# flash4242/Promptable-Counterfactual-GAN

Hardware: AMD Instinct MI355X
Metric: images/sec (G+D step) MNIST-28 cDCGAN bs512 @1/2/4/8 MI355X; % MFMA roofline (higher is better)
Workload: dtype f32

## Files before the change

### promptable-counterfactual-gan_amd/csrc/conv_igemm.hip

```cpp
#include <string.h>
#include <array>
#include <map>
#include <mutex>
#include "conv_loaders.h"
#include "conv_pixtab.h"
#include "conv_cliptab.h"
#include "thin_conv.h"

namespace pcg {
namespace {

__device__ __forceinline__ int wave_id() { return __builtin_amdgcn_readfirstlane((int)(threadIdx.x >> 6)); }

__device__ __forceinline__ void prio_entry(const ConvP& p) { if (p.edge_prio & 1) __builtin_amdgcn_s_setprio(3); }
__device__ __forceinline__ void prio_epilogue(const ConvP& p) { if (p.edge_prio & 2) __builtin_amdgcn_s_setprio(3); }

__device__ __forceinline__ int epi_group_off(const ConvP& p, int m_block) {
  return p.epi.group_rows > 0 ? __builtin_amdgcn_readfirstlane(m_block / p.epi.group_rows) * p.N : 0;
}

template <class Cfg, bool XF, bool CLIP = false>
__global__ void __launch_bounds__(IG_THREADS, Cfg::MINW) conv_fwd_kernel(ConvP p) {
  extern __shared__ __attribute__((aligned(16))) float smem[];
  prio_entry(p);
// ... 1782 lines not shown
      const int M = g->B * g->OH * g->OW, N = g->KH * g->KW * g->Cin, kt = ceil_div(g->Cout, IG_BK), tiles = ceil_div(M, 128) * ceil_div(N, 128);
      SkPlan sk{};
      say("%s", "GEMM + col2im: ");
      if (have && plan_sk_shape(tiles, kt, &sk)) say("stream-K: %d whole tiles + %d tiles x %d k-tiles over %d ranges", sk.dp_tiles, sk.sk_tiles, kt, sk.sk_blocks);
      else say("128x128 tiles: %d", tiles);
    } else {
      DgradPhases ph{};
      int maxMp = 0;
      const int nph = build_phases(g, &ph, &maxMp);
      const int N = g->Cin, tilesN = ceil_div(N, N > 64 ? 128 : 64);
      bool uniform = true;
      for (int i = 0; i < nph; ++i)
        uniform = uniform && ph.p[i].Mp == ph.p[0].Mp && ph.p[i].nth * ph.p[i].ntw == ph.p[0].nth * ph.p[0].ntw && ph.p[i].nth > 0 && ph.p[i].ntw > 0;
      SkNPlan sn{};
      SkPlan sk{};
      say("%d phase%s: ", nph, nph == 1 ? "" : "s");
      if (N > 64 && have && !uniform && plan_skn_shape(ph, nph, 128, tilesN, g->Cout, &sn))
        say("stream-K over unequal phases: %d tiles, %d k-tile iterations over %d ranges", sn.tile0[nph], sn.total, sn.blocks);
      else if (N > 64 && have && uniform && nph > 0 &&
               plan_sk_shape(ceil_div(maxMp, 128) * tilesN * nph, ph.p[0].nth * ph.p[0].ntw * ceil_div(g->Cout, IG_BK), &sk))
        say("stream-K: %d whole tiles + %d tiles over %d ranges", sk.dp_tiles, sk.sk_tiles, sk.sk_blocks);
      else say("%s tiles: %d per phase", N > 64 ? "128x128" : "128x64", ceil_div(maxMp, 128) * tilesN);
    }
  } else {
    const WgradPlan w = plan_wgrad(g);
    SkPlan sk{};
    if (!w.narrow && !w.wide192 && w.tiles > 96 && have && plan_sk_shape(w.tiles, w.ktiles_total, &sk))
      say("stream-K: %d whole tiles + %d tiles x %d k-tiles over %d ranges, dw written by the epilogue", sk.dp_tiles, sk.sk_tiles, w.ktiles_total, sk.sk_blocks);
    else if (!w.narrow && !w.wide192 && w.tiles > 96 && w.splits == 1 && sk_mode() != 0) say("128x128 tiles: %d, dw written by the epilogue", w.tiles);
    else say("%s tiles: %d x %d K-slices of %d k-tiles (slabs + slab_reduce)", w.wide192 ? "64x192" : w.narrow ? "64x128" : "128x128", w.tiles, w.splits, w.ktiles_per_split);
  }
  snprintf(out, out_bytes, "%s", buf);
  return PCG_OK;
}

extern "C" int pcg_conv_pad_clip_query(const pcg_conv_geom* g, int32_t op, int32_t groups, int32_t assume_scratch, int32_t* taken,
                                       int32_t* order, int32_t* tile_rows, double* predicted) {
  if (int e = check_geom(g)) return e;
  PCG_REQUIRE((op == 0 || op == 1) && groups >= 1, "pcg_conv_pad_clip_query: bad arguments");
  const int have = assume_scratch && sk_mode() != 0 ? 1 : 0;
  ClipPlan cp{false, 0, 0, 1.0};
  if (mfma_layer(g) && op == 0) {
    const int M = g->B * g->OH * g->OW, N = g->Cout, kt = g->KH * g->KW * ceil_div(g->Cin, IG_BK);
    const FwdPlan f = plan_fwd(g, have);
    const bool t64 = fwd_use_t64(M, N, f.splits);
    SkPlan sk{};
    const bool plain = f.splits == 1 && !(N > 64 && !t64 && have && plan_sk_shape(ceil_div(M, 128) * ceil_div(N, 128), kt, &sk));
    cp = clip_fwd_plan(g, groups, t64, plain);
  } else if (mfma_layer(g) && g->stride <= 2 && !dgrad_as_gemm(g, have)) {
    DgradPhases ph{};
    int maxMp = 0;
    const int nph = build_phases(g, &ph, &maxMp);
    SkPlan sk{};
    const bool plain = nph == 4 && !(g->Cin > 64 && have && plan_sk_shape(ceil_div(maxMp, 128) * ceil_div(g->Cin, 128) * nph, 4 * ceil_div(g->Cout, IG_BK), &sk));
    const uint32_t w_bytes = (uint32_t)((int64_t)g->Cout * g->KH * g->KW * g->Cin * 4);
    cp = clip_dgrad_plan(g, groups, dgrad_interleaved(w_bytes, ph, nph), plain);
  }
  if (taken) *taken = cp.take && cliptab_of(g) ? 1 : 0;
  if (order) *order = cp.order;
  if (tile_rows) *tile_rows = cp.bm;
  if (predicted) *predicted = cp.ratio;
  return PCG_OK;
}

extern "C" int pcg_tune_set(const char* name, int32_t value) {
  PCG_REQUIRE(name != nullptr, "pcg_tune_set: null name");
  if (!strcmp(name, "korder")) g_tune.korder = value;
  else if (!strcmp(name, "edge_prio")) g_tune.edge_prio = value;
  else if (!strcmp(name, "dgrad_swz3")) g_tune.dgrad_swz3 = value;
  else if (!strcmp(name, "wgrad_rounds")) g_tune.wgrad_rounds = value;
  else if (!strcmp(name, "wgrad_order")) g_tune.wgrad_order = value;
  else if (!strcmp(name, "dgrad_interleave")) g_tune.dgrad_interleave = value;
  else if (!strcmp(name, "fwd_splits")) g_tune.fwd_splits = value;
  else if (!strcmp(name, "stream_k")) g_tune.stream_k = value;
  else if (!strcmp(name, "sk_blocks")) g_tune.sk_blocks = value;
  else if (!strcmp(name, "dgrad_gemm")) g_tune.dgrad_gemm = value;
  else if (!strcmp(name, "t64")) g_tune.t64 = value;
  else if (!strcmp(name, "wgrad_pixtab")) g_tune.wgrad_pixtab = value;
  else if (!strcmp(name, "pad_clip")) g_tune.pad_clip = value;
  else if (!strcmp(name, "pad_clip_dgrad")) {
    PCG_REQUIRE(value >= -1 && value <= 2, "pcg_tune_set: pad_clip_dgrad is 0, 1 or 2 (-1: built-in), not %d", (int)value);
    g_tune.pad_clip_dgrad = value;
  }
  else {
    set_error("pcg_tune_set: unknown switch '%s' (korder, edge_prio, dgrad_swz3, wgrad_rounds, wgrad_order, dgrad_interleave, fwd_splits, "
              "stream_k, sk_blocks, dgrad_gemm, t64); the loader switches wgrad_pixtab, pad_clip and pad_clip_dgrad are accepted as well", name);
    return PCG_ERR_INVALID;
  }
  return PCG_OK;
}

extern "C" int pcg_debug_stamp_buffer(void* buf, int64_t bytes) {
  g_tune.stamps = static_cast<unsigned long long*>(buf);
  g_tune.stamp_slots = buf ? (int)(bytes / 16) : 0;
#ifdef PCG_CLOCK_STAMP
  return 1;
#else
  return 0;
#endif
}
```

### promptable-counterfactual-gan_amd/csrc/thin_conv.h

```cpp
#pragma once
#include "pcg_common.h"

namespace pcg {

inline bool thin_is_cin(const pcg_conv_geom* g) { return g->Cin <= 3; }
inline bool thin_is_cout(const pcg_conv_geom* g) { return g->Cout <= 3 && !thin_is_cin(g); }

struct ThinBnIn { const float* mean; const float* invstd; const float* gamma; const float* beta; int act; float slope; int groups; };
bool thin_conv_bnin_full_ok(const pcg_conv_geom* g, int groups);
int thin_conv_fwd(const pcg_conv_geom* g, const float* x, const float* w, const float* bias, float* y, void* ws,
                  size_t ws_bytes, hipStream_t s, int act = PCG_ACT_NONE, float slope = 0.f, const ThinBnIn* bnin = nullptr);
struct ThinXf { const float* scale; const float* shift; float neg; };
bool thin_conv_xf_ok(const pcg_conv_geom* g);
int thin_conv_dgrad(const pcg_conv_geom* g, const float* dy, const float* w, const float* bias_x, float* dx, void* ws,
                    size_t ws_bytes, hipStream_t s, int act = PCG_ACT_NONE, float slope = 0.f, const ThinXf* xf = nullptr);
size_t thin_conv_fwd_workspace_bytes(const pcg_conv_geom* g);
size_t thin_conv_dgrad_workspace_bytes(const pcg_conv_geom* g);
size_t thin_conv_wgrad_workspace_bytes(const pcg_conv_geom* g);
int thin_conv_wgrad(const pcg_conv_geom* g, const float* x, const float* dy, float* dw, int accumulate, void* ws,
                    size_t ws_bytes, hipStream_t s, const ThinXf* xf = nullptr, const ThinBnIn* bnin = nullptr);

bool thin_conv_fwd_bnbwd_ok(const pcg_conv_geom* g);
size_t thin_conv_fwd_bnbwd_workspace_bytes(const pcg_conv_geom* g);
int thin_conv_fwd_bnbwd(const pcg_conv_geom* g, const float* x, const float* w, const float* z, const float* mean, const float* invstd,
                        const float* gamma, const float* beta, int act, float slope, float* dz, float* dgamma, float* dbeta, int accumulate,
                        void* ws, size_t ws_bytes, hipStream_t s);

bool thin_conv_dgrad_mask_ok(const pcg_conv_geom* g);
int thin_conv_dgrad_mask(const pcg_conv_geom* g, const float* dy, const float* w, const float* a_below, int act, float slope, float* dx,
                         hipStream_t s);

bool thin_conv_dgrad_bnbwd_full_ok(const pcg_conv_geom* g, int groups);
size_t thin_conv_dgrad_bnbwd_full_workspace_bytes(const pcg_conv_geom* g, int groups);
int thin_conv_dgrad_bnbwd_full(const pcg_conv_geom* g, const float* dy, const float* w, const float* z, const float* mean, const float* invstd,
                               const float* gamma, const float* beta, int act, float slope, float* dz, float* dgamma, float* dbeta, int accumulate,
                               int groups, void* ws, size_t ws_bytes, hipStream_t s);

int launch_slab_reduce(const float* slab, float* dw, size_t n, size_t slab_stride, int nslabs, int accumulate, hipStream_t s, bool deferrable = false);

int slab_defer_begin(hipStream_t s);
int slab_defer_flush(hipStream_t s);
int slab_defer_pending();

}
```

### promptable-counterfactual-gan_amd/csrc/thin_conv.hip

```cpp
#include "thin_conv.h"
#include <cstdlib>

namespace pcg {
namespace {

struct ThinP {
  const float* thin;
  const float* wide;
  const float* w;
  const float* bias;
  float* out;
  int act; float slope;
  const float* xf_scale; const float* xf_shift; float xf_neg;
  const float* mask_src; float mask_neg;
  int B, TH, TW, Cs, WH, WW, C;
  int KH, KW, stride, pad, transposed;
  int wsS, wsT, wsC;
  int IH_, IW_;
  int QH, QW;
  int npix;
  FastDiv dIW, dIH, dCQ;
};

__device__ __forceinline__ bool tap_map(const ThinP& p, int ph, int pw, int kh, int kw, int& qh, int& qw) {
  if (!p.transposed) {
    qh = ph * p.stride - p.pad + kh;
    qw = pw * p.stride - p.pad + kw;
  } else {
    const int th = ph + p.pad - kh, tw = pw + p.pad - kw;
    if (th < 0 || tw < 0) return false;
    if (p.stride == 1) { qh = th; qw = tw; }
    else if (p.stride == 2) { if ((th | tw) & 1) return false; qh = th >> 1; qw = tw >> 1; }
    else { if (th % p.stride || tw % p.stride) return false; qh = th / p.stride; qw = tw / p.stride; }
  }
  return (unsigned)qh < (unsigned)p.QH && (unsigned)qw < (unsigned)p.QW;
}

__device__ __forceinline__ void stage_weights(const ThinP& p, float* Wl) {
  const int TT = p.KH * p.KW * p.Cs;
  for (int i = threadIdx.x; i < TT * p.C; i += blockDim.x) {
    const int t = i / p.C, c = i - t * p.C;
    const int tap = t / p.Cs, cs = t - tap * p.Cs;
    Wl[i] = p.w[(size_t)cs * p.wsS + (size_t)tap * p.wsT + (size_t)c * p.wsC];
  }
  __syncthreads();
}

__global__ void __launch_bounds__(256) thin_expand_kernel(ThinP p) {
  extern __shared__ __attribute__((aligned(16))) float Wl[];
  stage_weights(p, Wl);
  const int CQ = p.C >> 2;
  const uint32_t total = (uint32_t)p.npix * (uint32_t)CQ;
  const float4* bias4 = reinterpret_cast<const float4*>(p.bias);
  float4* out4 = reinterpret_cast<float4*>(p.out);
  for (uint32_t idx = blockIdx.x * 256u + threadIdx.x; idx < total; idx += gridDim.x * 256u) {
    uint32_t pix, cq, t, pw, b, ph;
    p.dCQ.divmod(idx, pix, cq);
    p.dIW.divmod(pix, t, pw);
    p.dIH.divmod(t, b, ph);
    float4 acc = p.bias ? bias4[cq] : make_float4(0.f, 0.f, 0.f, 0.f);
    for (int kh = 0; kh < p.KH; ++kh)
      for (int kw = 0; kw < p.KW; ++kw) {
        int qh, qw;
        if (!tap_map(p, (int)ph, (int)pw, kh, kw, qh, qw)) continue;
        const float* sp = p.thin + (size_t)(((int)b * p.TH + qh) * p.TW + qw) * p.Cs;
        const float* wl = Wl + (size_t)((kh * p.KW + kw) * p.Cs) * p.C + 4 * cq;
        for (int cs = 0; cs < p.Cs; ++cs) {
          const float sv = sp[cs];
          const float4 w4 = *reinterpret_cast<const float4*>(wl + (size_t)cs * p.C);
          acc.x = fmaf(sv, w4.x, acc.x); acc.y = fmaf(sv, w4.y, acc.y);
          acc.z = fmaf(sv, w4.z, acc.z); acc.w = fmaf(sv, w4.w, acc.w);
        }
      }
    if (p.act != PCG_ACT_NONE) {
      acc.x = act_neg_scale(acc.x, p.slope); acc.y = act_neg_scale(acc.y, p.slope);
      acc.z = act_neg_scale(acc.z, p.slope); acc.w = act_neg_scale(acc.w, p.slope);
    }
    out4[idx] = acc;
  }
}

__global__ void __launch_bounds__(256) thin_reduce_kernel(ThinP p) {
  extern __shared__ __attribute__((aligned(16))) float Wl[];
  stage_weights(p, Wl);
  const int CQ = p.C >> 2;
  const int l16 = threadIdx.x & 15, grp = threadIdx.x >> 4;
  for (uint32_t pix = blockIdx.x * 16u + grp; pix < (uint32_t)p.npix; pix += gridDim.x * 16u) {
// ... 429 lines not shown
}

bool is_pow2(int v) { return v > 0 && (v & (v - 1)) == 0; }

bool rows_plan(const ThinP& p, RowsP& rp, size_t* patch_bytes, int px_per_thread = 16, size_t max_patch_bytes = (size_t)ROWS_MAXP * 256 * sizeof(float)) {
  const bool direct = !p.transposed;
  if (!direct && p.stride != 1) return false;
  const int CQ = p.C / 4;
  if (p.C % 4 || CQ > 256 || !is_pow2(CQ)) return false;
  if (p.IH_ * p.IW_ < 64) return false;
  if ((int64_t)p.B * p.TH * p.TW * p.Cs * 4 >= (1ll << 31)) return false;
  const int PL = 256 / CQ;
  int R;
  if (px_per_thread == 16) {
    int target = PL * 16;
    if (target < 256) target = 256;
    R = (target + p.IW_ - 1) / p.IW_;
  } else {
    R = PL * px_per_thread / p.IW_;
    if (R < 1) return false;
  }
  if (R > p.IH_) R = p.IH_;
  rp.s = direct ? p.stride : 1;
  rp.flip = direct ? 0 : 1;
  rp.qh_off = direct ? -p.pad : p.pad - p.KH + 1;
  rp.qw_off = direct ? -p.pad : p.pad - p.KW + 1;
  rp.R = R;
  rp.upi = (p.IH_ + R - 1) / R;
  rp.nunits = p.B * rp.upi;
  rp.PH = (R - 1) * rp.s + p.KH;
  rp.PW = (p.IW_ - 1) * rp.s + p.KW;
  rp.dUPI = FastDiv((uint32_t)rp.upi);
  rp.dPWC = FastDiv((uint32_t)(rp.PW * p.Cs));
  rp.dCS = FastDiv((uint32_t)p.Cs);
  *patch_bytes = (size_t)rp.PH * rp.PW * p.Cs * sizeof(float);
  return *patch_bytes <= max_patch_bytes;
}

int fill_common(ThinP& p, const pcg_conv_geom* g, bool cin_thin, bool iter_on_output) {
  p.B = g->B; p.KH = g->KH; p.KW = g->KW; p.stride = g->stride; p.pad = g->pad;
  const int T = g->KH * g->KW;
  if (cin_thin) {
    p.TH = g->IH; p.TW = g->IW; p.Cs = g->Cin; p.WH = g->OH; p.WW = g->OW; p.C = g->Cout;
    p.wsS = 1; p.wsT = g->Cin; p.wsC = T * g->Cin;
  } else {
    p.TH = g->OH; p.TW = g->OW; p.Cs = g->Cout; p.WH = g->IH; p.WW = g->IW; p.C = g->Cin;
    p.wsS = T * g->Cin; p.wsT = g->Cin; p.wsC = 1;
  }
  p.transposed = iter_on_output ? 0 : 1;
  if (iter_on_output) { p.IH_ = g->OH; p.IW_ = g->OW; p.QH = g->IH; p.QW = g->IW; }
  else { p.IH_ = g->IH; p.IW_ = g->IW; p.QH = g->OH; p.QW = g->OW; }
  p.npix = g->B * p.IH_ * p.IW_;
  p.dIW = FastDiv((uint32_t)p.IW_); p.dIH = FastDiv((uint32_t)p.IH_); p.dCQ = FastDiv((uint32_t)(p.C / 4));
  PCG_REQUIRE(p.C % 4 == 0, "thin conv: wide channel count %d must be a multiple of 4", p.C);
  PCG_REQUIRE(p.Cs >= 1 && p.Cs <= 3, "thin conv: thin channel count %d not in 1..3", p.Cs);
  PCG_REQUIRE((int64_t)p.npix * (p.C / 4) < (1ll << 31), "thin conv: problem too large for 32-bit indexing");
  return PCG_OK;
}

unsigned rows_expand_blocks(int nunits) {
  static const int cap = [] { const char* e = getenv("PCG_ROWS_EXPAND_BLOCKS"); const int v = e ? atoi(e) : 0; return v > 0 ? v : 1024; }();
  return (unsigned)(nunits < cap ? nunits : cap);
}

size_t lds_weight_bytes(const ThinP& p) { return (size_t)p.KH * p.KW * p.Cs * p.C * sizeof(float); }

bool fast_ok(const ThinP& p) {
  return p.Cs == 1 && p.stride <= 2 && p.KH * p.KW <= 16 && p.C % 16 == 0 && lds_weight_bytes(p) <= 64 * 1024;
}

int launch_expand(ThinP& p, hipStream_t s) {
  const size_t smem = lds_weight_bytes(p);
  PCG_REQUIRE(smem <= 64 * 1024, "thin conv: weight image %zu B exceeds 64 KB of LDS", smem);
  const bool k44 = p.KH == 4 && p.KW == 4, k33 = p.KH == 3 && p.KW == 3, k11 = p.KH == 1 && p.KW == 1;
  RowsP rp{};
  size_t patch_bytes = 0;
  if ((k44 || k33) && (k33 || p.Cs == 1) && rows_plan(p, rp, &patch_bytes)) {
    const size_t two = 2 * ((patch_bytes + 15) & ~(size_t)15), sm = smem > two ? smem : two;
    const uint32_t thin_bytes = (uint32_t)((int64_t)p.B * p.TH * p.TW * p.Cs * 4);
    const unsigned blocks = rows_expand_blocks(rp.nunits);
    static const int mfma_on = [] { const char* e = getenv("PCG_EXPAND_MFMA"); return e ? atoi(e) : 1; }();
    if (mfma_on && p.C == 64 && (((uintptr_t)p.out | (uintptr_t)p.mask_src) & 15) == 0) {
      const size_t sm2 = 2 * ((patch_bytes + 15) & ~(size_t)15);
      if (k44) hipLaunchKernelGGL((thin_rows_expand_mfma_kernel<4, 4, 1>), dim3(blocks), dim3(256), sm2, s, p, rp, thin_bytes);
      else if (p.Cs == 1) hipLaunchKernelGGL((thin_rows_expand_mfma_kernel<3, 3, 1>), dim3(blocks), dim3(256), sm2, s, p, rp, thin_bytes);
      else if (p.Cs == 2) hipLaunchKernelGGL((thin_rows_expand_mfma_kernel<3, 3, 2>), dim3(blocks), dim3(256), sm2, s, p, rp, thin_bytes);
      else hipLaunchKernelGGL((thin_rows_expand_mfma_kernel<3, 3, 3>), dim3(blocks), dim3(256), sm2, s, p, rp, thin_bytes);
      return launch_status("thin_rows_expand_mfma_kernel");
    }
#define PCG_ROWS_EXPAND_CASE(KH_, KW_, CS_)                                                                                  \
    if (p.KH == KH_ && p.Cs == CS_) {                                                                                         \
      hipLaunchKernelGGL((thin_rows_expand_kernel<KH_, KW_, CS_>), dim3(blocks), dim3(256), sm, s, p, rp, thin_bytes);      \
      return launch_status("thin_rows_expand_kernel");                                                                        \
    }
    PCG_ROWS_EXPAND_CASE(4, 4, 1)
    PCG_ROWS_EXPAND_CASE(3, 3, 1)
    PCG_ROWS_EXPAND_CASE(3, 3, 2)
    PCG_ROWS_EXPAND_CASE(3, 3, 3)
#undef PCG_ROWS_EXPAND_CASE
  }
  if (fast_ok(p) && (k44 || k33 || k11) && (int64_t)p.npix * (p.C / 16) < (1ll << 31)) {
    ThinP q = p;
    q.dCQ = FastDiv((uint32_t)(p.C / 16));
    const uint32_t thin_bytes = (uint32_t)((int64_t)p.B * p.TH * p.TW * 4);
    const uint64_t total = (uint64_t)p.npix * (p.C / 16);
    unsigned blocks = (unsigned)((total + 255) / 256);
    if (blocks > 8192) blocks = 8192;
    if (k44) hipLaunchKernelGGL((thin_expand16_kernel<4, 4>), dim3(blocks), dim3(256), smem, s, q, thin_bytes);
    else if (k33) hipLaunchKernelGGL((thin_expand16_kernel<3, 3>), dim3(blocks), dim3(256), smem, s, q, thin_bytes);
    else hipLaunchKernelGGL((thin_expand16_kernel<1, 1>), dim3(blocks), dim3(256), smem, s, q, thin_bytes);
    return launch_status("thin_expand16_kernel");
  }
  const uint64_t total = (uint64_t)p.npix * (p.C / 4);
  unsigned blocks = (unsigned)((total + 255) / 256);
  if (blocks > 4096) blocks = 4096;
  hipLaunchKernelGGL(thin_expand_kernel, dim3(blocks), dim3(256), smem, s, p);
  return launch_status("thin_expand_kernel");
}

bool fast32_ok(const ThinP& p) {
  return p.Cs >= 2 && p.Cs <= 3 && p.KH == 3 && p.KW == 3 && p.stride <= 2 && p.C % 16 == 0 && lds_weight_bytes(p) <= 64 * 1024;
}

size_t reduce_scratch_bytes(const ThinP& p) {
  if (fast32_ok(p)) {
    const int64_t b = (int64_t)p.B * p.WH * p.WW * 32 * 4;
    return b < (1ll << 31) ? (size_t)b : 0;
  }
  if (!fast_ok(p)) return 0;
  const int64_t b = (int64_t)p.B * p.WH * p.WW * 16 * 4;
  return b < (1ll << 31) ? (size_t)b : 0;
}

int launch_reduce(ThinP& p, void* ws, size_t ws_bytes, hipStream_t s) {
  const size_t smem = lds_weight_bytes(p);
  PCG_REQUIRE(smem <= 64 * 1024, "thin conv: weight image %zu B exceeds 64 KB of LDS", smem);
  const size_t need = reduce_scratch_bytes(p);
  PCG_REQUIRE(!p.xf_scale || !fast32_ok(p), "thin conv: input transforms only with one thin channel");
  if (need && ws && ws_bytes >= need && (((uintptr_t)ws) & 15) == 0 && fast32_ok(p)) {
    float* T = (float*)ws;
    ThinP q = p;
    q.npix = p.B * p.WH * p.WW;
    unsigned blocks = (unsigned)((q.npix + 15) / 16);
    if (blocks > 8192) blocks = 8192;
    uint32_t plane = 0;
    if (p.C == 64 && (((uintptr_t)p.wide) & 15) == 0) {
      unsigned mb = (unsigned)((q.npix + 127) / 128);
      if (mb > 4096) mb = 4096;
      hipLaunchKernelGGL((thin_tapdot64_mfma_kernel<2, false>), dim3(mb), dim3(256), 0, s, q, T);
      plane = (uint32_t)q.npix;
    } else if (p.Cs == 2) hipLaunchKernelGGL(thin_tapdot32_kernel<18>, dim3(blocks), dim3(256), smem, s, q, T);
    else hipLaunchKernelGGL(thin_tapdot32_kernel<27>, dim3(blocks), dim3(256), smem, s, q, T);
    if (int e = launch_status("thin_tapdot32_kernel")) return e;
    unsigned b2 = (unsigned)(((int64_t)p.npix * p.Cs + 255) / 256);
    if (b2 > 8192) b2 = 8192;
    hipLaunchKernelGGL(thin_col2im32_kernel, dim3(b2), dim3(256), 0, s, p, (const float*)T, (uint32_t)need, plane);
    return launch_status("thin_col2im32_kernel");
  }
  if (need && ws && ws_bytes >= need && (((uintptr_t)ws) & 15) == 0) {
    float* T = (float*)ws;
    ThinP q = p;
    q.npix = p.B * p.WH * p.WW;
    unsigned blocks = (unsigned)((q.npix + 15) / 16);
    if (blocks > 8192) blocks = 8192;
    const int nt = p.KH * p.KW;
    const bool mfma1 = p.C == 64, mfmaN = p.C % 64 == 0 && p.C > 64 && p.C <= TD64_MAX_C;
    uint32_t plane = 0;
    PCG_REQUIRE(!p.xf_scale || ((mfma1 || mfmaN) && nt <= 16 && (((uintptr_t)p.wide) & 15) == 0), "thin conv: an input transform needs the matrix-core tap-dot form");
    if ((mfma1 || mfmaN) && nt <= 16 && (((uintptr_t)p.wide) & 15) == 0) {
      unsigned mb = (unsigned)((q.npix + 127) / 128);
      if (mb > 4096) mb = 4096;
      if (mfma1) hipLaunchKernelGGL((thin_tapdot64_mfma_kernel<1, false>), dim3(mb), dim3(256), 0, s, q, T);
      else {
        if (mb > 1024) mb = 1024;
        hipLaunchKernelGGL((thin_tapdot64_mfma_kernel<1, true>), dim3(mb), dim3(256), (size_t)16 * (p.C + 4) * sizeof(float), s, q, T);
      }
      plane = (uint32_t)q.npix;
    } else if (nt == 16) hipLaunchKernelGGL(thin_tapdot_kernel<16>, dim3(blocks), dim3(256), smem, s, q, T);
    else if (nt == 9) hipLaunchKernelGGL(thin_tapdot_kernel<9>, dim3(blocks), dim3(256), smem, s, q, T);
    else if (nt == 1) hipLaunchKernelGGL(thin_tapdot_kernel<1>, dim3(blocks), dim3(256), smem, s, q, T);
    else goto generic;
    if (int e = launch_status("thin_tapdot_kernel")) return e;
    if (p.transposed && p.stride == 2 && p.KH == 4 && p.KW == 4 && p.IW_ % 4 == 0 && (((uintptr_t)p.out) & 15) == 0) {
      unsigned b4 = (unsigned)((p.npix / 4 + 255) / 256);
      if (b4 > 8192) b4 = 8192;
      hipLaunchKernelGGL(thin_col2im_s2k4_kernel, dim3(b4), dim3(256), 0, s, p, (const float*)T, (uint32_t)need, plane);
      return launch_status("thin_col2im_s2k4_kernel");
    }
    unsigned b2 = (unsigned)((p.npix + 255) / 256);
    if (b2 > 8192) b2 = 8192;
    hipLaunchKernelGGL(thin_col2im_kernel, dim3(b2), dim3(256), 0, s, p, (const float*)T, (uint32_t)need, plane);
    return launch_status("thin_col2im_kernel");
  }
generic:
  PCG_REQUIRE(!p.xf_scale, "thin conv: an input transform needs the matrix-core tap-dot form (workspace of pcg_conv2d_dgrad_workspace_bytes)");
  unsigned blocks = (unsigned)((p.npix + 15) / 16);
  if (blocks > 4096) blocks = 4096;
  hipLaunchKernelGGL(thin_reduce_kernel, dim3(blocks), dim3(256), smem, s, p);
  return launch_status("thin_reduce_kernel");
}

int rows_wgrad_blocks(const RowsP& rp) { return rp.nunits < 512 ? rp.nunits : 512; }
bool rows_wgrad_ok(const ThinP& p, const pcg_conv_geom* g, RowsP& rp, size_t* patch_bytes) {
  const bool k44 = g->KH == 4 && g->KW == 4 && p.Cs == 1, k33 = g->KH == 3 && g->KW == 3;
  return (k44 || k33) && rows_plan(p, rp, patch_bytes, ROWS_NPT, (size_t)ROWS_MAXP * 256 * sizeof(float));
}

struct ThinWgradPlan { int ppb, nblocks; };
ThinWgradPlan plan_thin_wgrad(int npix, int C) {
  ThinWgradPlan w;
  const int PL = 256 / (C / 4);
  int ppb = (npix + 1023) / 1024;
  const int min_ppb = PL * 8;
  if (ppb < min_ppb) ppb = min_ppb;
  w.ppb = ppb;
  w.nblocks = (npix + ppb - 1) / ppb;
  return w;
}

bool thin_wgrad_instantiated(const ThinP& p) {
  const bool k44 = p.KH == 4 && p.KW == 4, k33 = p.KH == 3 && p.KW == 3, k11 = p.KH == 1 && p.KW == 1;
  return p.C / 4 <= 256 && is_pow2(p.C / 4) && ((k44 && p.Cs == 1) || k33 || k11) && !(p.transposed && p.stride > 2);
}
ThinWgradPlan plan_thin_wgrad_any(int npix) {
  ThinWgradPlan w;
  int ppb = (npix + 1023) / 1024;
  if (ppb < 256) ppb = 256;
  w.ppb = ppb;
  w.nblocks = (npix + ppb - 1) / ppb;
  return w;
}

}

int launch_slab_reduce(const float* slab, float* dw, size_t n, size_t slab_stride, int nslabs, int accumulate, hipStream_t s, bool deferrable) {
  const bool vec = (n % 4 == 0) && (slab_stride % 4 == 0) && (((uintptr_t)slab | (uintptr_t)dw) & 15) == 0;
  if (deferrable && vec && g_slab_defer.on && s == g_slab_defer.stream && n / 4 < (1ull << 32) && slab_stride / 4 < (1ull << 32)) {
    SlabDefer& d = g_slab_defer;
    const size_t n4 = n / 4;
    bool clash = d.n == SLAB_MANY_MAX;
    for (int k = 0; k < d.n && !clash; ++k) clash = (const void*)d.m.e[k].dw == (const void*)dw;
    if (clash)
      if (int e = slab_defer_launch()) return e;
    const int wide = nslabs >= 64 && n4 <= 16 * 1024;
    d.m.e[d.n++] = SlabEntry{reinterpret_cast<const float4*>(slab), reinterpret_cast<float4*>(dw), (uint32_t)n4, (uint32_t)(slab_stride / 4), nslabs,
                             accumulate, wide};
    const unsigned blocks = (unsigned)(wide ? (n4 + 15) / 16 : (n4 + 255) / 256);
    if (blocks > d.max_blocks) d.max_blocks = blocks;
    return PCG_OK;
  }
  if (vec) {
    const size_t n4 = n / 4;
    if (nslabs >= 64 && n4 <= 16 * 1024) {
      hipLaunchKernelGGL(slab_reduce4_wide_kernel, dim3((unsigned)((n4 + 15) / 16)), dim3(256), 0, s, reinterpret_cast<const float4*>(slab),
                         reinterpret_cast<float4*>(dw), n4, slab_stride / 4, nslabs, accumulate);
      return launch_status("slab_reduce_kernel");
    }
    unsigned blocks = (unsigned)((n4 + 63) / 64);
    if (blocks > 4096) blocks = 4096;
    if (blocks == 0) blocks = 1;
    hipLaunchKernelGGL(slab_reduce4_kernel, dim3(blocks), dim3(64), 0, s, reinterpret_cast<const float4*>(slab),
                       reinterpret_cast<float4*>(dw), n4, slab_stride / 4, nslabs, accumulate);
  } else {
    unsigned blocks = (unsigned)((n + 255) / 256);
    if (blocks > 2048) blocks = 2048;
    if (blocks == 0) blocks = 1;
    hipLaunchKernelGGL(slab_reduce1_kernel, dim3(blocks), dim3(256), 0, s, slab, dw, n, slab_stride, nslabs, accumulate);
  }
  return launch_status("slab_reduce_kernel");
}

bool thin_conv_bnin_full_ok(const pcg_conv_geom* g, int groups) {
  if (!full_window(g) || groups < 1 || groups > 8 || g->B % groups || g->Cin % 4) return false;
  const int CQ = g->Cin / 4;
  return CQ <= 256 && 256 % CQ == 0 && (g->B / groups) % FULL_ROWS_DW == 0;
}
static FullXf full_xf_of(const pcg_conv_geom* g, const ThinBnIn* bi) {
  if (!bi || !bi->mean) return FullXf{nullptr, nullptr, nullptr, nullptr, 1.f, g->Cin, g->B};
  return FullXf{bi->mean, bi->invstd, bi->gamma, bi->beta, act_neg_of(bi->act, bi->slope), g->Cin, g->B / bi->groups};
}

int thin_conv_fwd(const pcg_conv_geom* g, const float* x, const float* w, const float* bias, float* y, void* ws,
                  size_t ws_bytes, hipStream_t s, int act, float slope, const ThinBnIn* bnin) {
  PCG_REQUIRE(!(bnin && bnin->mean) || (thin_conv_bnin_full_ok(g, bnin->groups) && (((uintptr_t)x | (uintptr_t)w) & 15) == 0),
              "thin conv forward: a BatchNorm input needs the full-window form (thin_conv_bnin_full_ok) and 16-byte aligned tensors");
  ThinP p{};
  p.act = act; p.slope = slope;
  const bool cin_thin = thin_is_cin(g);
  if (int e = fill_common(p, g, cin_thin, true)) return e;
  p.w = w; p.bias = bias; p.out = y;
  if (cin_thin) {
    p.thin = x;
    const bool fuse = act_is_cheap(act);
    p.act = fuse ? act : PCG_ACT_NONE; p.slope = act_neg_of(p.act, slope);
    if (int e = launch_expand(p, s)) return e;
    return fuse ? PCG_OK : pcg_act_fwd(y, (int64_t)g->B * g->OH * g->OW * g->Cout, act, slope, y, (pcg_stream_t)s);
  }
  p.wide = x;
  if (full_window(g) && (((uintptr_t)x | (uintptr_t)w) & 15) == 0) {
    const int L4 = g->KH * g->KW * g->Cin / 4;
    hipLaunchKernelGGL(thin_full_dot_kernel, dim3((unsigned)(g->B < 4096 ? g->B : 4096)), dim3(256), 0, s, reinterpret_cast<const float4*>(x),
                       reinterpret_cast<const float4*>(w), bias, y, g->B, L4, act, slope, full_xf_of(g, bnin));
    return launch_status("thin_full_dot_kernel");
  }
  return launch_reduce(p, ws, ws_bytes, s);
}

int launch_bn_bwd_finalize(const double* partial, int nblocks, int64_t rows, int C, const float* gamma, const float* invstd, float* coef,
                           float* dgamma, float* dbeta, int accumulate, hipStream_t s);

constexpr unsigned THIN_BN_BLOCKS = 2048;
size_t thin_conv_fwd_bnbwd_workspace_bytes(const pcg_conv_geom* g) {
  return (size_t)THIN_BN_BLOCKS * 2 * g->Cout * sizeof(double) + (size_t)3 * g->Cout * sizeof(float);
}
bool thin_conv_fwd_bnbwd_ok(const pcg_conv_geom* g) {
  if (!thin_is_cin(g) || g->Cin != 1 || !(g->KH == 4 && g->KW == 4)) return false;
  ThinP p{};
// ... 265 lines not shown
```

### promptable-counterfactual-gan_amd/csrc/thin_rows.inc

```

struct RowsP {
  int R, upi, nunits;
  int PH, PW;
  int s;
  int qh_off, qw_off;
  int flip;
  FastDiv dUPI, dPWC, dCS;
};

constexpr int ROWS_MAXP = 8;
struct PatchGather { int pr[ROWS_MAXP], pc[ROWS_MAXP]; };
__device__ __forceinline__ void patch_gather_init(const RowsP& rp, int PF, PatchGather& pg) {
#pragma unroll
  for (int j = 0; j < ROWS_MAXP; ++j) {
    const int i = threadIdx.x + 256 * j;
    uint32_t r, rem, c, cs;
    rp.dPWC.divmod((uint32_t)i, r, rem);
    rp.dCS.divmod(rem, c, cs);
    pg.pr[j] = i < PF ? (int)r : -(1 << 20);
    pg.pc[j] = ((rp.qw_off + (int)c) << 2) | (int)cs;
  }
}
template <int CS>
__device__ __forceinline__ void patch_issue(const ThinP& p, const RowsP& rp, thin_rsrc_t rs, const PatchGather& pg, int b, int r0,
// ... 17 lines not shown
template <int KH, int KW, int CS>
__global__ void __launch_bounds__(256) thin_rows_expand_kernel(ThinP p, RowsP rp, uint32_t thin_bytes) {
  constexpr int NT = KH * KW * CS;
  extern __shared__ __attribute__((aligned(16))) float smem_rows[];
  float* Wl = smem_rows;
  const int CQ = p.C >> 2, PL = 256 / CQ;
  const int cq = threadIdx.x % CQ, pl = threadIdx.x / CQ;
  for (int i = threadIdx.x; i < NT * p.C; i += 256) {
    const int t = i / p.C, c = i - t * p.C;
    const int tap = t / CS, cs = t - tap * CS;
    Wl[i] = p.w[(size_t)cs * p.wsS + (size_t)tap * p.wsT + (size_t)c * p.wsC];
  }
  __syncthreads();
  float4 w[NT];
#pragma unroll
  for (int t = 0; t < NT; ++t) w[t] = *reinterpret_cast<const float4*>(Wl + t * p.C + 4 * cq);
  const float4 bv = p.bias ? *reinterpret_cast<const float4*>(p.bias + 4 * cq) : make_float4(0.f, 0.f, 0.f, 0.f);
  const thin_rsrc_t rs = thin_rsrc(p.thin, thin_bytes);
  const FastDiv dIW = p.dIW;
  const int PF = rp.PH * rp.PW * CS, PFS = (PF + 3) & ~3;
  PatchGather pg;
  patch_gather_init(rp, PF, pg);
  float pv[ROWS_MAXP];
  int cur = 0;
  if ((int)blockIdx.x < rp.nunits) {
    uint32_t b, ur;
    rp.dUPI.divmod(blockIdx.x, b, ur);
    patch_issue<CS>(p, rp, rs, pg, (int)b, (int)ur * rp.R, pv);
  }
  __syncthreads();
  patch_put(smem_rows, pv, PF);
  __syncthreads();
  for (int unit = blockIdx.x; unit < rp.nunits; unit += gridDim.x) {
    uint32_t b, ur;
    rp.dUPI.divmod((uint32_t)unit, b, ur);
    const int r0 = (int)ur * rp.R;
    const int nxt = unit + (int)gridDim.x;
    if (nxt < rp.nunits) {
      uint32_t bn_, un_;
      rp.dUPI.divmod((uint32_t)nxt, bn_, un_);
      patch_issue<CS>(p, rp, rs, pg, (int)bn_, (int)un_ * rp.R, pv);
    }
    const float* patch = smem_rows + cur * PFS;
    int rows = p.IH_ - r0; if (rows > rp.R) rows = rp.R;
    const int np = rows * p.IW_;
    float4* o = reinterpret_cast<float4*>(p.out + ((size_t)((int)b * p.IH_ + r0) * p.IW_) * p.C) + cq;
    const float4* ms = p.mask_src ? reinterpret_cast<const float4*>(p.mask_src + ((size_t)((int)b * p.IH_ + r0) * p.IW_) * p.C) + cq : nullptr;
    for (int lp = pl; lp < np; lp += PL) {
      float4 mv = make_float4(1.f, 1.f, 1.f, 1.f);
      if (ms) mv = ms[(size_t)lp * CQ];
      uint32_t lh, pw;
      dIW.divmod((uint32_t)lp, lh, pw);
      const float* pp = patch + ((int)lh * rp.s * rp.PW + (int)pw * rp.s) * CS;
      float4 acc = bv;
#pragma unroll
      for (int kh = 0; kh < KH; ++kh)
#pragma unroll
        for (int kw = 0; kw < KW; ++kw) {
          const int khp = rp.flip ? KH - 1 - kh : kh, kwp = rp.flip ? KW - 1 - kw : kw;
#pragma unroll
          for (int cs = 0; cs < CS; ++cs) {
            const float sv = pp[(khp * rp.PW + kwp) * CS + cs];
            const float4 w4 = w[(kh * KW + kw) * CS + cs];
            acc.x = fmaf(sv, w4.x, acc.x); acc.y = fmaf(sv, w4.y, acc.y);
            acc.z = fmaf(sv, w4.z, acc.z); acc.w = fmaf(sv, w4.w, acc.w);
          }
        }
      if (p.act != PCG_ACT_NONE) {
        acc.x = act_neg_scale(acc.x, p.slope); acc.y = act_neg_scale(acc.y, p.slope);
        acc.z = act_neg_scale(acc.z, p.slope); acc.w = act_neg_scale(acc.w, p.slope);
      }
      if (ms) {
        acc.x *= mv.x > 0.f ? 1.f : p.mask_neg; acc.y *= mv.y > 0.f ? 1.f : p.mask_neg;
        acc.z *= mv.z > 0.f ? 1.f : p.mask_neg; acc.w *= mv.w > 0.f ? 1.f : p.mask_neg;
      }
      o[(size_t)lp * CQ] = acc;
    }
    if (nxt < rp.nunits) patch_put(smem_rows + (cur ^ 1) * PFS, pv, PF);
    __syncthreads();
    cur ^= 1;
  }
}

template <int KH, int KW, int CS>
__global__ void __launch_bounds__(256) thin_rows_expand_mfma_kernel(ThinP p, RowsP rp, uint32_t thin_bytes) {
  constexpr int NT = KH * KW * CS, KS = (NT + 3) / 4;
  static_assert(NT <= 32, "thin_rows_expand_mfma_kernel: at most 32 (tap, thin channel) pairs");
  extern __shared__ __attribute__((aligned(16))) float smem_rows[];
  __shared__ __attribute__((aligned(16))) float turn[4][16 * TD64_LD];
  const int lane = threadIdx.x & 63, wave = threadIdx.x >> 6;
  const int col = lane & 15, h = lane >> 4;
  float* S = turn[wave];
  float bw[KS][4];
#pragma unroll
  for (int ks = 0; ks < KS; ++ks)
#pragma unroll
    for (int nb = 0; nb < 4; ++nb) {
      const int kk = 4 * ks + h, tap = kk / CS, cs = kk - tap * CS;
      bw[ks][nb] = kk < NT ? p.w[(size_t)cs * p.wsS + (size_t)tap * p.wsT + (size_t)(16 * nb + col) * p.wsC] : 0.f;
    }
  float bv[4];
#pragma unroll
  for (int nb = 0; nb < 4; ++nb) bv[nb] = p.bias ? p.bias[16 * nb + col] : 0.f;
  int toff[KS];
#pragma unroll
  for (int ks = 0; ks < KS; ++ks) {
    const int kk = 4 * ks + h < NT ? 4 * ks + h : 0;
    const int tap = kk / CS, cs = kk - tap * CS;
    const int kh = tap / KW, kw = tap - kh * KW;
    const int khp = rp.flip ? KH - 1 - kh : kh, kwp = rp.flip ? KW - 1 - kw : kw;
    toff[ks] = (khp * rp.PW + kwp) * CS + cs;
  }
  const thin_rsrc_t rs = thin_rsrc(p.thin, thin_bytes);
  const FastDiv dIW = p.dIW;
  const int PF = rp.PH * rp.PW * CS, PFS = (PF + 3) & ~3;
  PatchGather pg;
  patch_gather_init(rp, PF, pg);
  float pv[ROWS_MAXP];
  int cur = 0;
  if ((int)blockIdx.x < rp.nunits) {
    uint32_t b, ur;
    rp.dUPI.divmod(blockIdx.x, b, ur);
    patch_issue<CS>(p, rp, rs, pg, (int)b, (int)ur * rp.R, pv);
  }
  patch_put(smem_rows, pv, PF);
  __syncthreads();
  for (int unit = blockIdx.x; unit < rp.nunits; unit += gridDim.x) {
    uint32_t b, ur;
    rp.dUPI.divmod((uint32_t)unit, b, ur);
    const int r0 = (int)ur * rp.R;
    const int nxt = unit + (int)gridDim.x;
    if (nxt < rp.nunits) {
      uint32_t bn_, un_;
      rp.dUPI.divmod((uint32_t)nxt, bn_, un_);
      patch_issue<CS>(p, rp, rs, pg, (int)bn_, (int)un_ * rp.R, pv);
    }
    const float* patch = smem_rows + cur * PFS;
    int rows = p.IH_ - r0; if (rows > rp.R) rows = rp.R;
    const int np = rows * p.IW_;
    float4* o = reinterpret_cast<float4*>(p.out + ((size_t)((int)b * p.IH_ + r0) * p.IW_) * 64);
    const float4* ms = p.mask_src ? reinterpret_cast<const float4*>(p.mask_src + ((size_t)((int)b * p.IH_ + r0) * p.IW_) * 64) : nullptr;
    for (int lp0 = 16 * wave; lp0 < np; lp0 += 64) {
      int lp = lp0 + col; if (lp >= np) lp = np - 1;
      uint32_t lh, pw;
      dIW.divmod((uint32_t)lp, lh, pw);
      const float* pp = patch + ((int)lh * rp.s * rp.PW + (int)pw * rp.s) * CS;
      float a[KS];
#pragma unroll
      for (int ks = 0; ks < KS; ++ks) a[ks] = pp[toff[ks]];
      thin_f32x4 acc[4];
#pragma unroll
      for (int nb = 0; nb < 4; ++nb) acc[nb] = thin_f32x4{bv[nb], bv[nb], bv[nb], bv[nb]};
#pragma unroll
      for (int ks = 0; ks < KS; ++ks)
#pragma unroll
        for (int nb = 0; nb < 4; ++nb) acc[nb] = __builtin_amdgcn_mfma_f32_16x16x4f32(a[ks], bw[ks][nb], acc[nb], 0, 0, 0);
#pragma unroll
      for (int nb = 0; nb < 4; ++nb)
#pragma unroll
        for (int i = 0; i < 4; ++i) {
          float v = acc[nb][i];
          if (p.act != PCG_ACT_NONE) v = act_neg_scale(v, p.slope);
          S[(4 * h + i) * TD64_LD + 16 * nb + col] = v;
        }
#pragma unroll
      for (int j = 0; j < 4; ++j) {
        const int px = 4 * j + h;
        float4 v = *reinterpret_cast<const float4*>(S + px * TD64_LD + 4 * col);
        if (lp0 + px < np) {
          if (ms) {
            const float4 mv = ms[(size_t)(lp0 + px) * 16 + col];
            v.x *= mv.x > 0.f ? 1.f : p.mask_neg; v.y *= mv.y > 0.f ? 1.f : p.mask_neg;
            v.z *= mv.z > 0.f ? 1.f : p.mask_neg; v.w *= mv.w > 0.f ? 1.f : p.mask_neg;
          }
          o[(size_t)(lp0 + px) * 16 + col] = v;
        }
      }
    }
    if (nxt < rp.nunits) patch_put(smem_rows + (cur ^ 1) * PFS, pv, PF);
    __syncthreads();
    cur ^= 1;
  }
}

struct ThinBnBwd {
  const float* z; const float* mean; const float* invstd; const float* gamma; const float* beta; const float* coef;
  float neg;
  double* partial;
};

template <int KH, int KW, int CS, bool APPLY>
__global__ void __launch_bounds__(256) thin_rows_expand_bn_kernel(ThinP p, RowsP rp, uint32_t thin_bytes, ThinBnBwd bn) {
  constexpr int NT = KH * KW * CS;
  extern __shared__ __attribute__((aligned(16))) float smem_rows[];
  __shared__ double red[256];
  float* Wl = smem_rows;
  const int CQ = p.C >> 2, PL = 256 / CQ;
  const int cq = threadIdx.x % CQ, pl = threadIdx.x / CQ;
  for (int i = threadIdx.x; i < NT * p.C; i += 256) {
    const int t = i / p.C, c = i - t * p.C;
    const int tap = t / CS, cs = t - tap * CS;
    Wl[i] = p.w[(size_t)cs * p.wsS + (size_t)tap * p.wsT + (size_t)c * p.wsC];
  }
  __syncthreads();
  float4 w[NT];
#pragma unroll
  for (int t = 0; t < NT; ++t) w[t] = *reinterpret_cast<const float4*>(Wl + t * p.C + 4 * cq);
  float sc[4], sh[4], mu[4], is[4], k0[4], k1[4], k2[4];
#pragma unroll
  for (int e = 0; e < 4; ++e) {
    const int c = 4 * cq + e;
    mu[e] = bn.mean[c]; is[e] = bn.invstd[c];
    bn_fold(bn.gamma[c], bn.beta[c], mu[e], is[e], sc[e], sh[e]);
    k0[e] = APPLY ? bn.coef[c] : 0.f; k1[e] = APPLY ? bn.coef[p.C + c] : 0.f; k2[e] = APPLY ? bn.coef[2 * p.C + c] : 0.f;
  }
  double s1[4] = {0.0, 0.0, 0.0, 0.0}, s2[4] = {0.0, 0.0, 0.0, 0.0};
  const thin_rsrc_t rs = thin_rsrc(p.thin, thin_bytes);
  const FastDiv dIW = p.dIW;
  const int PF = rp.PH * rp.PW * CS, PFS = (PF + 3) & ~3;
  PatchGather pg;
  patch_gather_init(rp, PF, pg);
  float pv[ROWS_MAXP];
  int cur = 0;
  if ((int)blockIdx.x < rp.nunits) {
    uint32_t b, ur;
    rp.dUPI.divmod(blockIdx.x, b, ur);
    patch_issue<CS>(p, rp, rs, pg, (int)b, (int)ur * rp.R, pv);
  }
  __syncthreads();
  patch_put(smem_rows, pv, PF);
  __syncthreads();
  for (int unit = blockIdx.x; unit < rp.nunits; unit += gridDim.x) {
    uint32_t b, ur;
    rp.dUPI.divmod((uint32_t)unit, b, ur);
    const int r0 = (int)ur * rp.R;
    const int nxt = unit + (int)gridDim.x;
    if (nxt < rp.nunits) {
      uint32_t bn_, un_;
      rp.dUPI.divmod((uint32_t)nxt, bn_, un_);
      patch_issue<CS>(p, rp, rs, pg, (int)bn_, (int)un_ * rp.R, pv);
    }
    const float* patch = smem_rows + cur * PFS;
    int rows = p.IH_ - r0; if (rows > rp.R) rows = rp.R;
    const int np = rows * p.IW_;
    const size_t base4 = ((size_t)((int)b * p.IH_ + r0) * p.IW_) * CQ + cq;
    const float4* zp = reinterpret_cast<const float4*>(bn.z) + base4;
    float4* o = reinterpret_cast<float4*>(p.out) + base4;
    for (int lp = pl; lp < np; lp += PL) {
      const float4 zv = zp[(size_t)lp * CQ];
      uint32_t lh, pw;
      dIW.divmod((uint32_t)lp, lh, pw);
// ... 401 lines not shown
```

Before: 53310.

## Permute thin-expand MFMA operand mapping so accumulators form float4 stores directly

Adds a QUAD variant of the thin-conv rows-expand MFMA kernel. It permutes the output-channel mapping of the weights and bias (4*col+nb) and the pixel row assignment, so each lane's accumulator elements already form a contiguous float4 for one pixel. This removes the per-wave LDS transpose buffer and its write/read round trip. Dropping that buffer also lets the kernel declare a higher occupancy launch bound, and the grid is capped at 512 blocks by default. The path is on by default and can be switched off with an env var or a tune switch; correctness depends on the permuted row/column mapping matching the MFMA output layout.

```diff
diff --git a/promptable-counterfactual-gan_amd/csrc/conv_igemm.hip b/promptable-counterfactual-gan_amd/csrc/conv_igemm.hip
--- a/promptable-counterfactual-gan_amd/csrc/conv_igemm.hip
+++ b/promptable-counterfactual-gan_amd/csrc/conv_igemm.hip
@@ -1888,9 +1888,10 @@
     PCG_REQUIRE(value >= -1 && value <= 2, "pcg_tune_set: pad_clip_dgrad is 0, 1 or 2 (-1: built-in), not %d", (int)value);
     g_tune.pad_clip_dgrad = value;
   }
+  else if (!strcmp(name, "thin_quad")) thin_quad_set(value);
   else {
     set_error("pcg_tune_set: unknown switch '%s' (korder, edge_prio, dgrad_swz3, wgrad_rounds, wgrad_order, dgrad_interleave, fwd_splits, "
-              "stream_k, sk_blocks, dgrad_gemm, t64); the loader switches wgrad_pixtab, pad_clip and pad_clip_dgrad are accepted as well", name);
+              "stream_k, sk_blocks, dgrad_gemm, t64); the loader switches wgrad_pixtab, pad_clip and pad_clip_dgrad and the thin-layer switch thin_quad are accepted as well", name);
     return PCG_ERR_INVALID;
   }
   return PCG_OK;
diff --git a/promptable-counterfactual-gan_amd/csrc/thin_conv.h b/promptable-counterfactual-gan_amd/csrc/thin_conv.h
--- a/promptable-counterfactual-gan_amd/csrc/thin_conv.h
+++ b/promptable-counterfactual-gan_amd/csrc/thin_conv.h
@@ -36,6 +36,8 @@
                                const float* gamma, const float* beta, int act, float slope, float* dz, float* dgamma, float* dbeta, int accumulate,
                                int groups, void* ws, size_t ws_bytes, hipStream_t s);
 
+void thin_quad_set(int value);
+
 int launch_slab_reduce(const float* slab, float* dw, size_t n, size_t slab_stride, int nslabs, int accumulate, hipStream_t s, bool deferrable = false);
 
 int slab_defer_begin(hipStream_t s);
diff --git a/promptable-counterfactual-gan_amd/csrc/thin_conv.hip b/promptable-counterfactual-gan_amd/csrc/thin_conv.hip
--- a/promptable-counterfactual-gan_amd/csrc/thin_conv.hip
+++ b/promptable-counterfactual-gan_amd/csrc/thin_conv.hip
@@ -3,6 +3,12 @@
 
 namespace pcg {
 namespace {
+
+int g_thin_quad = -1;
+bool thin_quad_on() {
+  static const int env = [] { const char* e = getenv("PCG_THIN_QUAD"); return e ? atoi(e) : 1; }();
+  return (g_thin_quad >= 0 ? g_thin_quad : env) != 0;
+}
 
 struct ThinP {
   const float* thin;
@@ -598,10 +604,19 @@
     static const int mfma_on = [] { const char* e = getenv("PCG_EXPAND_MFMA"); return e ? atoi(e) : 1; }();
     if (mfma_on && p.C == 64 && (((uintptr_t)p.out | (uintptr_t)p.mask_src) & 15) == 0) {
       const size_t sm2 = 2 * ((patch_bytes + 15) & ~(size_t)15);
-      if (k44) hipLaunchKernelGGL((thin_rows_expand_mfma_kernel<4, 4, 1>), dim3(blocks), dim3(256), sm2, s, p, rp, thin_bytes);
-      else if (p.Cs == 1) hipLaunchKernelGGL((thin_rows_expand_mfma_kernel<3, 3, 1>), dim3(blocks), dim3(256), sm2, s, p, rp, thin_bytes);
-      else if (p.Cs == 2) hipLaunchKernelGGL((thin_rows_expand_mfma_kernel<3, 3, 2>), dim3(blocks), dim3(256), sm2, s, p, rp, thin_bytes);
-      else hipLaunchKernelGGL((thin_rows_expand_mfma_kernel<3, 3, 3>), dim3(blocks), dim3(256), sm2, s, p, rp, thin_bytes);
+      if (thin_quad_on()) {
+        static const bool grid_env = getenv("PCG_ROWS_EXPAND_BLOCKS") != nullptr;
+        const unsigned blocks = grid_env ? rows_expand_blocks(rp.nunits) : (unsigned)(rp.nunits < 512 ? rp.nunits : 512);
+        if (k44) hipLaunchKernelGGL((thin_rows_expand_mfma_kernel<4, 4, 1, true>), dim3(blocks), dim3(256), sm2, s, p, rp, thin_bytes);
+        else if (p.Cs == 1) hipLaunchKernelGGL((thin_rows_expand_mfma_kernel<3, 3, 1, true>), dim3(blocks), dim3(256), sm2, s, p, rp, thin_bytes);
+        else if (p.Cs == 2) hipLaunchKernelGGL((thin_rows_expand_mfma_kernel<3, 3, 2, true>), dim3(blocks), dim3(256), sm2, s, p, rp, thin_bytes);
+        else hipLaunchKernelGGL((thin_rows_expand_mfma_kernel<3, 3, 3, true>), dim3(blocks), dim3(256), sm2, s, p, rp, thin_bytes);
+        return launch_status("thin_rows_expand_mfma_kernel(quad)");
+      }
+      if (k44) hipLaunchKernelGGL((thin_rows_expand_mfma_kernel<4, 4, 1, false>), dim3(blocks), dim3(256), sm2, s, p, rp, thin_bytes);
+      else if (p.Cs == 1) hipLaunchKernelGGL((thin_rows_expand_mfma_kernel<3, 3, 1, false>), dim3(blocks), dim3(256), sm2, s, p, rp, thin_bytes);
+      else if (p.Cs == 2) hipLaunchKernelGGL((thin_rows_expand_mfma_kernel<3, 3, 2, false>), dim3(blocks), dim3(256), sm2, s, p, rp, thin_bytes);
+      else hipLaunchKernelGGL((thin_rows_expand_mfma_kernel<3, 3, 3, false>), dim3(blocks), dim3(256), sm2, s, p, rp, thin_bytes);
       return launch_status("thin_rows_expand_mfma_kernel");
     }
 #define PCG_ROWS_EXPAND_CASE(KH_, KW_, CS_)                                                                                  \
@@ -749,6 +764,8 @@
 
 }
 
+void thin_quad_set(int value) { g_thin_quad = value; }
+
 int launch_slab_reduce(const float* slab, float* dw, size_t n, size_t slab_stride, int nslabs, int accumulate, hipStream_t s, bool deferrable) {
   const bool vec = (n % 4 == 0) && (slab_stride % 4 == 0) && (((uintptr_t)slab | (uintptr_t)dw) & 15) == 0;
   if (deferrable && vec && g_slab_defer.on && s == g_slab_defer.stream && n / 4 < (1ull << 32) && slab_stride / 4 < (1ull << 32)) {
diff --git a/promptable-counterfactual-gan_amd/csrc/thin_rows.inc b/promptable-counterfactual-gan_amd/csrc/thin_rows.inc
--- a/promptable-counterfactual-gan_amd/csrc/thin_rows.inc
+++ b/promptable-counterfactual-gan_amd/csrc/thin_rows.inc
@@ -123,26 +123,31 @@
   }
 }
 
-template <int KH, int KW, int CS>
-__global__ void __launch_bounds__(256) thin_rows_expand_mfma_kernel(ThinP p, RowsP rp, uint32_t thin_bytes) {
+template <int KH, int KW, int CS, bool QUAD>
+__global__ void __launch_bounds__(256, QUAD && KH * KW * CS <= 16 ? 4 : 1) thin_rows_expand_mfma_kernel(ThinP p, RowsP rp, uint32_t thin_bytes) {
   constexpr int NT = KH * KW * CS, KS = (NT + 3) / 4;
   static_assert(NT <= 32, "thin_rows_expand_mfma_kernel: at most 32 (tap, thin channel) pairs");
   extern __shared__ __attribute__((aligned(16))) float smem_rows[];
-  __shared__ __attribute__((aligned(16))) float turn[4][16 * TD64_LD];
   const int lane = threadIdx.x & 63, wave = threadIdx.x >> 6;
   const int col = lane & 15, h = lane >> 4;
-  float* S = turn[wave];
+  float* S = nullptr;
+  if constexpr (!QUAD) {
+    __shared__ __attribute__((aligned(16))) float turn[4][16 * TD64_LD];
+    S = turn[wave];
+  }
   float bw[KS][4];
 #pragma unroll
   for (int ks = 0; ks < KS; ++ks)
 #pragma unroll
     for (int nb = 0; nb < 4; ++nb) {
       const int kk = 4 * ks + h, tap = kk / CS, cs = kk - tap * CS;
-      bw[ks][nb] = kk < NT ? p.w[(size_t)cs * p.wsS + (size_t)tap * p.wsT + (size_t)(16 * nb + col) * p.wsC] : 0.f;
+      const int c = QUAD ? 4 * col + nb : 16 * nb + col;
+      bw[ks][nb] = kk < NT ? p.w[(size_t)cs * p.wsS + (size_t)tap * p.wsT + (size_t)c * p.wsC] : 0.f;
     }
   float bv[4];
 #pragma unroll
-  for (int nb = 0; nb < 4; ++nb) bv[nb] = p.bias ? p.bias[16 * nb + col] : 0.f;
+  for (int nb = 0; nb < 4; ++nb) bv[nb] = p.bias ? p.bias[QUAD ? 4 * col + nb : 16 * nb + col] : 0.f;
+  const int prow = QUAD ? 4 * (col & 3) + (col >> 2) : col;
   int toff[KS];
 #pragma unroll
   for (int ks = 0; ks < KS; ++ks) {
@@ -182,7 +187,7 @@
     float4* o = reinterpret_cast<float4*>(p.out + ((size_t)((int)b * p.IH_ + r0) * p.IW_) * 64);
     const float4* ms = p.mask_src ? reinterpret_cast<const float4*>(p.mask_src + ((size_t)((int)b * p.IH_ + r0) * p.IW_) * 64) : nullptr;
     for (int lp0 = 16 * wave; lp0 < np; lp0 += 64) {
-      int lp = lp0 + col; if (lp >= np) lp = np - 1;
+      int lp = lp0 + prow; if (lp >= np) lp = np - 1;
       uint32_t lh, pw;
       dIW.divmod((uint32_t)lp, lh, pw);
       const float* pp = patch + ((int)lh * rp.s * rp.PW + (int)pw * rp.s) * CS;
@@ -196,18 +201,29 @@
       for (int ks = 0; ks < KS; ++ks)
 #pragma unroll
         for (int nb = 0; nb < 4; ++nb) acc[nb] = __builtin_amdgcn_mfma_f32_16x16x4f32(a[ks], bw[ks][nb], acc[nb], 0, 0, 0);
-#pragma unroll
-      for (int nb = 0; nb < 4; ++nb)
-#pragma unroll
-        for (int i = 0; i < 4; ++i) {
-          float v = acc[nb][i];
-          if (p.act != PCG_ACT_NONE) v = act_neg_scale(v, p.slope);
-          S[(4 * h + i) * TD64_LD + 16 * nb + col] = v;
-        }
+      if constexpr (!QUAD) {
+#pragma unroll
+        for (int nb = 0; nb < 4; ++nb)
+#pragma unroll
+          for (int i = 0; i < 4; ++i) {
+            float v = acc[nb][i];
+            if (p.act != PCG_ACT_NONE) v = act_neg_scale(v, p.slope);
+            S[(4 * h + i) * TD64_LD + 16 * nb + col] = v;
+          }
+      }
 #pragma unroll
       for (int j = 0; j < 4; ++j) {
         const int px = 4 * j + h;
-        float4 v = *reinterpret_cast<const float4*>(S + px * TD64_LD + 4 * col);
+        float4 v;
+        if constexpr (QUAD) {
+          v = make_float4(acc[0][j], acc[1][j], acc[2][j], acc[3][j]);
+          if (p.act != PCG_ACT_NONE) {
+            v.x = act_neg_scale(v.x, p.slope); v.y = act_neg_scale(v.y, p.slope);
+            v.z = act_neg_scale(v.z, p.slope); v.w = act_neg_scale(v.w, p.slope);
+          }
+        } else {
+          v = *reinterpret_cast<const float4*>(S + px * TD64_LD + 4 * col);
+        }
         if (lp0 + px < np) {
           if (ms) {
             const float4 mv = ms[(size_t)(lp0 + px) * 16 + col];
```

Result: no change. 53280, median of 2 (-0.1%).
